# uurl/hivemq-mqtt-tensorflow-kafka-realtime-iot-machine-learning-training-inference

Hardware: AMD Instinct MI355X
Metric: sensor-rows/sec (autoencoder train) + p50 per-event inference µs at 1/2/4/8 MI355X (higher is better)
Workload: dtype bf16

## Files before the change

### hivemq-mqtt-tensorflow-kafka-realtime-iot-machine-learning-training-inference_amd/csrc/include/sml_ops.h

```cpp
#pragma once
#include <hip/hip_runtime.h>
#include <stdint.h>

namespace sml {

int ae_nslot();
int ae_train_blocks_per_cu();
int ae_nparam();
int ae_waves_per_block();
int ae_train_grid(int64_t n, int max_blocks);
hipError_t ae_train_launch(const float* x, int64_t n, int64_t ld, const float* scale, const float* shift,
                           const float* params, float* partials, int64_t* iter, const int64_t* cursor,
                           const int* dims, const int* acts, float l1, int want_acc, int grid, const uint8_t* xpack,
                           hipStream_t stream, int* grid_used,
                           unsigned xpack_live = 0);
hipError_t ae_forward_launch(const float* x, int64_t n, int64_t ld, const float* scale, const float* shift,
                             const float* params, float* recon, float* score, uint8_t* flag, float threshold,
                             const int* dims, const int* acts, int max_blocks, hipStream_t stream,
                             float* metrics = nullptr);
hipError_t reduce_adam_launch(const float* partials, int G, int S, int nparam, float* grad_out, float* params,
                              float* m, float* v, const int64_t* iter, float lr, float beta1, float beta2, float eps,
                              float gscale, float* metrics_acc, int flags, int64_t* cursor, int64_t cursor_step,
                              int64_t cursor_ring, hipStream_t stream);
int slab_adam_columns(int S);
// ... 90 lines not shown
                                 const float* h0, const float* c0, const float* W, const float* Uw, const float* b,
                                 float* dh0, float* dc0, float* partials, int64_t B, int T, int IN, int act,
                                 int dh_last_only, int64_t x_seq, int frag, hipStream_t st);
inline int lstm_fused_bwd_slabs(int64_t B, int U, int IN, bool dx, bool x_bf16, bool dh_last_only) {
  return lstm_split_applies(U, IN, dx, x_bf16, dh_last_only) ? lstm_split_grid(B) : lstm_fused_slabs(B, U, dx);
}
int lstm_head_partials(int64_t n, int N);
hipError_t lstm_head_launch(const void* h, int64_t ldh, const float* W, const float* b, const float* y, int64_t ldy,
                            void* dh, int64_t n, int N, float gscale, float* part, float* grad, const int* map,
                            float* acc, float* out, float div0, float div1, int64_t* counter, hipStream_t st);
bool lstm_fused_frag_supported(int U, int IN, bool x_bf16, bool want_dx);

hipError_t pack_tiles_argmax_launch(const float* x, int64_t n, int64_t ld, int D, const float* scale,
                                    const float* shift, uint8_t* out, hipStream_t stream,
                                    const int64_t* index = nullptr, uint64_t perm_key = 0, int64_t perm_n = 0,
                                    uint64_t live_mask = 0);
hipError_t perm_indices_launch(int64_t* out, int64_t start, int64_t count, int64_t n, uint64_t key,
                               hipStream_t stream);
hipError_t row_argmax_launch(const float* x, int64_t n, int64_t ld, int D, const float* scale, const float* shift,
                             uint8_t* out, hipStream_t stream);

hipError_t mlp_fwd_launch(const void* x, int x_u8, int64_t ldx, const float* W, const float* b, float* y, int M,
                          int K, int N, int relu, float keep, uint32_t seed, uint32_t step, hipStream_t st);
hipError_t mlp_bwd_data_launch(const float* dz, const float* W, const float* h, float* dh, int M, int N1, int N2,
                               float inv_keep, hipStream_t st);
hipError_t mlp_wgrad_launch(const void* x, int x_u8, int64_t ldx, const float* dy, float* out, int B, int K, int N,
                            hipStream_t st);
hipError_t mlp_dropout_mask_launch(float* out, int M, int N, float keep, uint32_t seed, uint32_t step,
                                   hipStream_t st);

int lstm_ref_train_params();
// ... 76 lines not shown
```

### hivemq-mqtt-tensorflow-kafka-realtime-iot-machine-learning-training-inference_amd/csrc/kernels/ae_fused.hip

```cpp
#include <cstdlib>

#include "sml_common.h"
#include "sml_adam.h"

using namespace sml;

namespace {

constexpr int WAVES = 4;
constexpr int OFF1 = 0, OFF2 = 512, OFF3 = 768, OFF4 = 1024;
constexpr int NPARAM = 1536;
constexpr int NSLOT = 1540;
constexpr int SLAB_BYTES = WAVES * NSLOT * 4;

struct AEArgs {
  const float* x;
  int64_t n;
  int64_t ld;
  const float* scale;
  const float* shift;
  const float* params;
  float* partials;
  int64_t* iter;
  const int64_t* cursor;
// ... 620 lines not shown
    dz4r1[u] = lds_transpose(dz4b1[u], scr + 9 * 512, c, g);
  }
  if constexpr (U == 1) {
    xr0[1] = xr1[1] = dz1r[1] = h1r[1] = dz2r[1] = h2r[1] = dz3r[1] = h3r[1] = dz4r0[1] = dz4r1[1] = zb;
  }
  acc1[0] = mfma32(xr0[0], xr0[1], dz1r[0], dz1r[1], acc1[0]);
  acc1[1] = mfma32(xr1[0], xr1[1], dz1r[0], dz1r[1], acc1[1]);
  acc2 = mfma32(h1r[0], h1r[1], dz2r[0], dz2r[1], acc2);
  acc3 = mfma32(h2r[0], h2r[1], dz3r[0], dz3r[1], acc3);
  acc4[0] = mfma32(h3r[0], h3r[1], dz4r0[0], dz4r0[1], acc4[0]);
  acc4[1] = mfma32(h3r[0], h3r[1], dz4r1[0], dz4r1[1], acc4[1]);
}

constexpr unsigned kLiveCardata = 0x3FFFFu & ~((1u << 0) | (1u << 2) | (1u << 4) | (1u << 5));
__host__ __device__ constexpr bool cm_dead(int f) { return f == 0 || f == 2 || f == 4 || f == 5; }
__device__ __forceinline__ int cm_off(int g) { return g < 2 ? 0 : g == 2 ? 16 : 32; }
__device__ __forceinline__ f32x4 cm_row_x(const char* row, int g) {
  typedef __attribute__((address_space(3))) const f32x2_t lds_f2;
  const f32x2_t a = *(lds_f2*)(row + cm_off(g)), b = *(lds_f2*)(row + cm_off(g) + 8);
  return f32x4{a[0], g == 0 ? a[0] : a[1], b[0], g == 0 ? a[1] : b[1]};
}
__device__ __forceinline__ f32x4 cm_zero_dead(f32x4 x, int g) {
  return f32x4{g < 2 ? 0.f : x[0], g == 1 ? 0.f : x[1], g == 0 ? 0.f : x[2], x[3]};
}

struct FragsP {
  bf16x4 w1t;
  bf16x4 w1u[2];
  bf16x4 w2t[2];
  bf16x4 w3t;
  bf16x4 w4t[2];
  bf16x4 w4u;
  bf16x4 w4b[2];
  bf16x4 w4bu;
  bf16x4 w3b;
  bf16x4 w2b[2];
  s16x8 w1a[2], w2a, w4ba, w4bua;
  s16x8 w1s;
};
// ... 121 lines not shown
    s1 = base + pin * w + 16 + 4 * (out - 16);
    s2 = base + (pin + 8) * w + 16 + 8 + 4 * (out - 16);
    return;
  }
  s1 = base + pin * w + out;
  s2 = base + (pin + 8) * w + out + (l3 ? 8 : 0);
}

__device__ __forceinline__ void tr_write(bf16x4 v, char* slot, int c, int g) {
  *(lds_bf16x4*)(slot + tr_wr_off(c, g)) = v;
}
__device__ __forceinline__ bf16x4 tr_read(char* slot, int c, int g) {
  return __builtin_amdgcn_ds_read_tr16_b64_v4i16((lds_bf16x4*)(slot + tr_rd_off(c, g)));
}

template <int PACK, int DC, bool TP, int TS = 10, int NP = 1, int XP = 0, bool RX = false, bool CM = false>
__device__ __forceinline__ void train_pair_packed(const AEArgs& a, const FragsP& F, char* scr, int c, int g,
                                                  const f32x4 (&xf)[NP][2][2], const float (&xup)[NP],
                                                  const int (&ix)[NP][2], f32x4 acc1[2], f32x4& acc2, f32x4& acc3,
                                                  f32x4 acc4[2], f32x4& acc2b, f32x4& acc4b, float& sq, float& ab,
                                                  float& corr, float& rows, const char* const* xring = nullptr) {
  static_assert(PACK == PACK_REF && DC == 18, "reference model, D = 18 (outputs 16, 17 packed as UP)");
  static_assert(NP == 1 || NP == 2, "one or two pairs per iteration");
  const f32x4 zero4 = {0.f, 0.f, 0.f, 0.f};
  const bf16x4 zb = {0, 0, 0, 0};
  const bool pad_lane = (g == 3);
  const bool lo = c < 8;
  auto stand_in = [](int p, int u) { return TP && p == NP - 1 && u == 1; };
  constexpr bool EW = XP == 1 || XP == 3, MA = XP >= 1, TRM = XP == 2;
  bf16x4 ident;
#pragma unroll
  for (int j = 0; j < 4; ++j) ident[j] = bfbits(4 * g + j == c ? 1.0f : 0.0f);
  auto mfma_tr = [&](bf16x4 v) -> bf16x4 { return pack4(mfma16(v, ident, zero4)); };

  bf16x4 xb0[NP][2], h1b[NP][2], xub[NP];
  f32x4 h1[NP][2], y[NP][2], z1[NP][2], l1s[NP][2];
#pragma unroll
  for (int p = 0; p < NP; ++p) {
#pragma unroll
    for (int u = 0; u < 2; ++u) xb0[p][u] = pack4(xf[p][u][0]);
    xub[p] = pack4(f32x4{xup[p], g == 0 ? 1.0f : 0.0f, 0.f, 0.f});
    if constexpr (EW) {
      tr_write(xb0[p][0], scr + (p * 10 + 0) * 512, c, g);
      tr_write(xb0[p][1], scr + (p * 10 + 1) * 512, c, g);
      tr_write(xub[p], scr + (p * 10 + 2) * 512, c, g);
    }
  }
#pragma unroll
  for (int p = 0; p < NP; ++p) {
    if constexpr (MA) {
      const bf16x4 xu0 = pack4(f32x4{g < 2 ? xup[p] : 0.f, g == 0 ? 1.0f : 0.0f, 0.f, 0.f});
      const bf16x4 xu1 = pack4(f32x4{g >= 2 ? xup[p] : 0.f, g == 0 ? 1.0f : 0.0f, 0.f, 0.f});
      z1[p][0] = mfma32a(F.w1s, xb0[p][0], xu0, zero4);
      z1[p][1] = mfma32a(F.w1s, xb0[p][1], xu1, zero4);
    } else {
      z1[p][0] = mfma32a(F.w1a[0], xb0[p][0], xub[p], zero4);
      z1[p][1] = mfma32a(F.w1a[1], xub[p], xb0[p][1], zero4);
    }
  }
#pragma unroll
  for (int p = 0; p < NP; ++p)
#pragma unroll
    for (int u = 0; u < 2; ++u) {
#pragma unroll
      for (int i = 0; i < 4; ++i) h1[p][u][i] = tanh_exp2(z1[p][u][i]);
      h1b[p][u] = pack4(h1[p][u]);
      if constexpr (EW) tr_write(h1b[p][u], scr + (p * 10 + 3 + u) * 512, c, g);
// ... 22 lines not shown
  for (int p = 0; p < NP; ++p) z3[p] = mfma16(F.w3t, h2b[p], zero4);
#pragma unroll
  for (int p = 0; p < NP; ++p) {
#pragma unroll
    for (int i = 0; i < 4; ++i) h3[p][i] = tanh_exp2(z3[p][i]);
    h3b[p] = pack4(h3[p]);
    if constexpr (EW) tr_write(h3b[p], scr + (p * 10 + 6) * 512, c, g);
  }
  f32x4 dz4[NP][2], z4[NP][2], z4u[NP];
  float dz4up[NP], yup[NP];
  f32x4 xl[NP][2];
  float xul[NP];
#pragma unroll
  for (int p = 0; p < NP; ++p) {
    if constexpr (RX) {
      typedef __attribute__((address_space(3))) const f32x2_t lds_f2;
      typedef __attribute__((address_space(3))) const float lds_f;
      constexpr int DR = CM ? 14 : 18, SLOTB = 64 * DR + 16;
#pragma unroll
      for (int u = 0; u < 2; ++u) {
        if constexpr (CM) {
          xl[p][u] = cm_row_x(xring[p] + u * SLOTB + c * 4 * DR, g);
        } else {
          const char* row = xring[p] + u * SLOTB + c * 4 * 18 + 16 * g;
          const f32x2_t v0 = *(lds_f2*)row, v1 = *(lds_f2*)(row + 8);
          xl[p][u] = f32x4{v0[0], v0[1], v1[0], v1[1]};
        }
      }
      xul[p] = *(lds_f*)(xring[p] + c * 4 * DR + 4 * (DR - 2 + (g & 1)) + (g >= 2 ? SLOTB : 0));
    } else {
#pragma unroll
      for (int u = 0; u < 2; ++u) xl[p][u] = xf[p][u][0];
      xul[p] = xup[p];
    }
    if constexpr (CM) {
#pragma unroll
      for (int u = 0; u < 2; ++u) xl[p][u] = cm_zero_dead(xl[p][u], g);
    }
  }
#pragma unroll
  for (int p = 0; p < NP; ++p) {
#pragma unroll
    for (int u = 0; u < 2; ++u) z4[p][u] = mfma16(F.w4t[u], h3b[p], zero4);
    z4u[p] = mfma16(F.w4u, h3b[p], zero4);
  }
#pragma unroll
  for (int p = 0; p < NP; ++p) {
#pragma unroll
    for (int u = 0; u < 2; ++u)
#pragma unroll
      for (int i = 0; i < 4; ++i) {
        y[p][u][i] = relu_fast(z4[p][u][i]);
        float e = y[p][u][i] - xl[p][u][i];
        if (stand_in(p, u)) e = 0.f;
        sq = fmaf(e, e, sq);
        dz4[p][u][i] = y[p][u][i] > 0.f ? e : 0.f;
      }
    yup[p] = relu_fast(z4u[p][0]);
    float eup = yup[p] - xul[p];
    if (TP && p == NP - 1) eup = g < 2 ? eup : 0.f;
    sq = fmaf(eup, eup, sq);
    dz4up[p] = yup[p] > 0.f ? eup : 0.f;
  }
  if (a.want_acc) {
#pragma unroll
    for (int p = 0; p < NP; ++p) {
      const int iy = row_argmax_up_pair(y[p][0], y[p][1], yup[p], g);
      const int sel = -(g & 1);
      const int ixs = (ix[p][0] & ~sel) | (ix[p][1] & sel);
      corr += (((TP && p == NP - 1) ? g == 0 : g < 2) && iy == ixs) ? 1.f : 0.f;
    }
  }
  rows += (g == 0) ? (TP ? 2.f * NP - 1.f : 2.f * NP) : 0.f;

  bf16x4 dz4b[NP][2], dz1b[NP][2], dz4bu[NP], dz3b[NP], dz2b[NP];
  f32x4 d3[NP], d2[NP];
#pragma unroll
  for (int p = 0; p < NP; ++p) {
#pragma unroll
    for (int u = 0; u < 2; ++u) dz4b[p][u] = pack4(dz4[p][u]);
    dz4bu[p] = pack4(f32x4{dz4up[p], 0.f, 0.f, 0.f});
  }
#pragma unroll
  for (int p = 0; p < NP; ++p) {
    d3[p] = mfma32a(F.w4ba, dz4b[p][0], dz4b[p][1], zero4);
    d3[p] = mfma32a(F.w4bua, dz4bu[p], zb, d3[p]);
  }
#pragma unroll
// ... 200 lines not shown
        if (lane < nl2) glds16(src + 1024, voff, dst + 1024);
      };
      constexpr int CH = XM == 3 ? 8 : 1;
      auto next_tile = [&](int64_t t) -> int64_t {
        if constexpr (CH == 1) return t + stride;
        return ((t + 1) & (CH - 1)) ? t + 1 : t + 1 + (stride - 1) * CH;
      };
      const int64_t t0 = ufirst * CH;
      if constexpr (ILP >= 2) {
        static_assert((XM == 1 || (XM == 0 && ILP == 3)) && CH == 1 && PF >= 3,
                      "tile pairs: tile-packed ring (or raw rows, packed pairs), plain order");
        auto ring_tile = [&](int slot, f32x4 xf[2], int& ix) {
          typedef __attribute__((address_space(3))) const unsigned char lds_u8;
          if constexpr (XM == 1) ix = (int)*(lds_u8*)(ring + slot * slotb + (slotb - 16) + c);
          if constexpr (CMP) {
            xf[0] = cm_row_x(ring + slot * slotb + c * 4 * DR, g);
            xf[1] = f32x4{0.f, 0.f, 0.f, 0.f};
            return;
          }
          if constexpr (ILP == 3) {
            typedef __attribute__((address_space(3))) const f32x2_t lds_f2;
            const char* row = ring + slot * slotb + c * 4 * a.D + 16 * g;
            const f32x2_t v0 = *(lds_f2*)row, v1 = *(lds_f2*)(row + 8);
            xf[0] = f32x4{v0[0], v0[1], v1[0], v1[1]};
            xf[1] = f32x4{0.f, 0.f, 0.f, 0.f};
            return;
          }
          ring_x(a, ring + slot * slotb, c, g, xf);
#pragma unroll
          for (int j = 0; j < 4; ++j) xf[1][j] = (live_hi<DC>(j) && 16 + 4 * g + j < DC) ? xf[1][j] : 0.f;
        };
        static_assert(ILP != 3 || PF % 2 == 0, "pairs start on even ring slots");
        const int up_off = c * 4 * DR + 4 * (DR - 2 + (g & 1)) + (g >= 2 ? slotb : 0);
        auto ring_up = [&](int slot) -> float {
          typedef __attribute__((address_space(3))) const float lds_f;
          return *(lds_f*)(ring + slot * slotb + up_off);
        };
        if constexpr (ILP == 3) {
          constexpr int PS = PF / 2, NVP = CMP ? 2 : 3;
          const int pairb = 2 * slotb;
          const int nl3 = (pairb - (CMP ? 1024 : 2048)) >> 4;
          const int64_t npairs = nfull >> 1;
          auto issue_pair = [&](int64_t pi, int ps) {
            pi = pi < npairs ? pi : npairs - 1;
            const char* src = (XM == 1 ? reinterpret_cast<const char*>(a.xpack) : reinterpret_cast<const char*>(a.x)) +
                              pi * pairb;
            const unsigned dst = ring_lds + ps * pairb;
            glds16(src, voff, dst);
            if constexpr (CMP) {
              if (lane < nl3) glds16(src + 1024, voff, dst + 1024);
            } else {
              glds16(src + 1024, voff, dst + 1024);
              if (lane < nl3) glds16(src + 2048, voff, dst + 2048);
            }
          };
          static_assert(PS > NPW, "ring: at least one pair in flight");
          auto load_pair = [&](int slot, f32x4 (&xf)[2][2], float& xup, int (&ix)[2]) {
            ring_tile(2 * slot, xf[0], ix[0]);
            ring_tile(2 * slot + 1, xf[1], ix[1]);
            xup = ring_up(2 * slot);
            if constexpr (XM == 0) {
              typedef __attribute__((address_space(3))) const f32x4 lds_f4;
              typedef __attribute__((address_space(3))) const float lds_f;
              const f32x4 nsc = *(lds_f4*)(norm + 16 * g), nsh = *(lds_f4*)(norm + 128 + 16 * g);
              const int fu = 4 * (16 + (g & 1));
              const float usc = *(lds_f*)(norm + fu), ush = *(lds_f*)(norm + 128 + fu);
#pragma unroll
              for (int u = 0; u < 2; ++u)
#pragma unroll
                for (int j = 0; j < 4; ++j) xf[u][0][j] = fmaf(xf[u][0][j], nsc[j], nsh[j]);
              xup = fmaf(xup, usc, ush);
              ix[0] = ix[1] = a.want_acc ? row_argmax_up_pair_signed(xf[0][0], xf[1][0], xup, g) : -1;
            }
          };
          int64_t pp = ufirst;
#pragma unroll
          for (int k = 0; k < PS - NPW; ++k) {
            issue_pair(pp, k);
            pp += stride;
          }
          int rs = 0, ws = PS - NPW;
          int64_t pi = ufirst;
          for (; pi + (NPW - 1) * stride < npairs; pi += NPW * stride) {
#pragma unroll
            for (int k = 0; k < NPW; ++k) {
              issue_pair(pp, ws);
              pp += stride;
              ws = ws + 1 == PS ? 0 : ws + 1;
            }
            asm volatile("s_waitcnt vmcnt(%0)" ::"n"(NVP * (PS - NPW)) : "memory");
            f32x4 xf[NPW][2][2];
            float xup[NPW];
            int ix[NPW][2];
            const char* xr[NPW];
#pragma unroll
            for (int k = 0; k < NPW; ++k) {
              load_pair(rs, xf[k], xup[k], ix[k]);
              xr[k] = ring + 2 * rs * slotb;
              rs = rs + 1 == PS ? 0 : rs + 1;
            }
            constexpr bool RX = XM == 1 && OCC >= 4;
            train_pair_packed<PACK, DC, false, TS, NPW, XP, RX, CMP>(a, FP, scr, c, g, xf, xup, ix, acc1, acc2, acc3,
                                                                     acc4, acc2b, acc4b, sq, ab, corr, rows, xr);
          }
          if (NPW == 2 && pi < npairs) {
            static_assert(NPW == 1 || PS - NPW - 1 >= 0, "ring depth");
            asm volatile("s_waitcnt vmcnt(%0)" ::"n"(NVP * (PS - NPW - 1)) : "memory");
            f32x4 xf[1][2][2];
            float xup[1];
            int ix[1][2];
            load_pair(rs, xf[0], xup[0], ix[0]);
            train_pair_packed<PACK, DC, false, TS, 1, XP, false, CMP>(a, FP, scr, c, g, xf, xup, ix, acc1, acc2, acc3,
                                                                      acc4, acc2b, acc4b, sq, ab, corr, rows);
          }
          asm volatile("s_waitcnt vmcnt(0)" ::: "memory");
        } else {
        int64_t tp = t0;
#pragma unroll
        for (int k = 0; k < PF - 2; ++k) {
          issue(tp, k);
          tp += stride;
        }
        int rd = 0, wr = PF - 2;
        int64_t t = t0;
        for (; t + stride < nfull; t += 2 * stride) {
          issue(tp, wr);
          issue(tp + stride, wr + 1 == PF ? 0 : wr + 1);
          tp += 2 * stride;
          asm volatile("s_waitcnt vmcnt(%0)" ::"n"(NV * (PF - 2)) : "memory");
          f32x4 xf[2][2];
// ... 498 lines not shown
  auto pair_grid = [&](int occ_pairs = 3) {
    static const int rounds = [] {
      const char* e = std::getenv("SML_AE_ROUNDS");
      const int r = e ? std::atoi(e) : 3;
      return r >= 1 && r <= 8 ? r : 3;
    }();
    set_grid(rounds * occ_pairs * device_cus());
  };
  if (pack == PACK_REF) {
    const bool xa_ok = xpack != nullptr && want_acc && (n & 15) == 0 &&
                       ((reinterpret_cast<uintptr_t>(xpack) & 15) == 0);
    static const int probe = [] {
      const char* e = std::getenv("SML_AE_XPROBE");
      return e ? std::atoi(e) : 0;
    }();
    const bool pairs_ok = ((n >> 4) & 1) == 0 && train_ilp() == 3 && dims[1] <= 15 && dims[2] <= 7 && dims[3] <= 7;
    const bool full = xpack_live == 0 || (D <= 31 && xpack_live == (1u << D) - 1u);
    const bool cm = !full && D == 18 && xpack_live == kLiveCardata;
    if (xpack != nullptr && !full && !cm) return hipErrorInvalidValue;
    const bool xpack_used = xa_ok && ring_ok && D == 18 && (cm ? pairs_ok : (train_ilp() == 2 || pairs_ok || occ == 4));
    if (xpack != nullptr && !xpack_used && (probe < 2 || cm)) return hipErrorInvalidValue;
    if (ring_ok && occ == 4 && D == 18 && want_acc && probe == 2)
      hipLaunchKernelGGL((ae_train_kernel<PACK_REF, true, 3, 4, 18, 2>), gd, bd, 0, stream, a);
    else if (ring_ok && occ == 4 && D == 18 && want_acc && probe == 3)
      hipLaunchKernelGGL((ae_train_kernel<PACK_REF, true, 3, 4, 18, 3>), gd, bd, 0, stream, a);
    else if (ring_ok && D == 18 && xa_ok && train_ilp() == 2) {
      pair_grid();
      hipLaunchKernelGGL((ae_train_kernel<PACK_REF, true, 6, 3, 18, 1, 2>), gd, bd, 0, stream, a);
    } else if (ring_ok && D == 18 && xa_ok && ((n >> 4) & 1) == 0 && train_ilp() == 3 && dims[1] <= 15 &&
               dims[2] <= 7 && dims[3] <= 7) {
// ... 118 lines not shown
```

### hivemq-mqtt-tensorflow-kafka-realtime-iot-machine-learning-training-inference_amd/csrc/kernels/preprocess.hip

```cpp
#include <algorithm>

#include "sml_common.h"

namespace {

constexpr int kThreads = 256;
constexpr int kWaves = kThreads / 64;
constexpr int kTilesPerWave = 8;
constexpr int kRowsPerGroup = 16 * kTilesPerWave;

__device__ __forceinline__ void wave_lds_sync() {
  asm volatile("s_waitcnt lgkmcnt(0)" ::: "memory");
  __builtin_amdgcn_wave_barrier();
}

__device__ __forceinline__ int64_t imin64(int64_t a, int64_t b) { return a < b ? a : b; }
__device__ __forceinline__ int64_t imax64(int64_t a, int64_t b) { return a > b ? a : b; }

__device__ __forceinline__ float4 ld4(const float* p) { return *reinterpret_cast<const float4*>(p); }

}

namespace sml {
__host__ __device__ __forceinline__ uint64_t perm_mix(uint64_t z) {
// ... 130 lines not shown

__device__ __forceinline__ void load_tables(float* s_sc, float* s_sh, int period, int D, const float* scale,
                                            const float* shift) {
  for (int p = threadIdx.x; p < period; p += kThreads) {
    const int col = p % D;
    s_sc[p] = scale ? scale[col] : 1.0f;
    s_sh[p] = scale ? shift[col] : 0.0f;
  }
}

template <int DT, bool CONTIG, int MODE>
__global__ __launch_bounds__(kThreads) void rows_group_kernel(const float* __restrict__ x, int64_t n, int64_t ld,
                                                              int Drt, const float* __restrict__ scale,
                                                              const float* __restrict__ shift,
                                                              uint8_t* __restrict__ out, RowSource src,
                                                              int vec2, uint64_t live) {
  const int D = DT > 0 ? DT : Drt;
  __shared__ int s_col[64];
  const int nlive = MODE == 2 ? __popcll(live) : D;
  if (MODE == 2 && threadIdx.x < 64) {
    int k = (int)threadIdx.x, col = 0;
    for (int f = 0; f < D; ++f)
      if ((live >> f) & 1) {
        if (k == 0) col = f;
        --k;
      }
    s_col[threadIdx.x] = col;
  }
  extern __shared__ __attribute__((aligned(16))) char smem[];
  const int period = 4 * D;
  float* s_sc = reinterpret_cast<float*>(smem);
  float* s_sh = s_sc + period;
  const int lane = threadIdx.x & 63, wid = threadIdx.x >> 6;
  const int srcw = src.gather() ? 2 * kRowsPerGroup : 0;
  float* stage = s_sh + period + wid * (kRowsPerGroup * D + 32 + srcw);
  uint8_t* s_arg = reinterpret_cast<uint8_t*>(stage + kRowsPerGroup * D);
  int64_t* s_src = reinterpret_cast<int64_t*>(stage + kRowsPerGroup * D + 32);
  load_tables(s_sc, s_sh, period, D, scale, shift);
  __syncthreads();
  const int tile_chunks = 4 * D;
  const int ctile_chunks = 4 * nlive;
// ... 49 lines not shown
  }
}

size_t rows_group_lds(int D, bool gather) {
  return (size_t)(8 * D + kWaves * (kRowsPerGroup * D + 32 + (gather ? 2 * kRowsPerGroup : 0))) * sizeof(float);
}

int stream_grid(int64_t groups_of_waves) {
  const int64_t cap = 256 * 8;
  return (int)std::max<int64_t>(1, std::min<int64_t>(cap, (groups_of_waves + kWaves - 1) / kWaves));
}

template <int MODE>
hipError_t launch_rows_group(const float* x, int64_t n, int64_t ld, int D, const float* scale, const float* shift,
                             uint8_t* out, hipStream_t stream, RowSource src = RowSource{nullptr, 0, 0, 0},
                             uint64_t live = 0) {
  const bool gather = src.index != nullptr || src.half > 0;
  const bool contig = !gather && ld == D && (reinterpret_cast<uintptr_t>(x) & 15) == 0;
  const int vec2 = (ld & 1) == 0 && (reinterpret_cast<uintptr_t>(x) & 7) == 0;
  const int64_t groups = (n + kRowsPerGroup - 1) / kRowsPerGroup;
  const dim3 grid(stream_grid(groups)), block(kThreads);
  const size_t lds = rows_group_lds(D, gather);
  if (lds > 160 * 1024) return hipErrorInvalidValue;
  if (lds > 65536) {
    hipError_t e = hipSuccess;
    if (D == 18 && contig)
      e = hipFuncSetAttribute(reinterpret_cast<const void*>(rows_group_kernel<18, true, MODE>),
                              hipFuncAttributeMaxDynamicSharedMemorySize, (int)lds);
    else if (contig)
      e = hipFuncSetAttribute(reinterpret_cast<const void*>(rows_group_kernel<0, true, MODE>),
                              hipFuncAttributeMaxDynamicSharedMemorySize, (int)lds);
    else if (D == 18)
      e = hipFuncSetAttribute(reinterpret_cast<const void*>(rows_group_kernel<18, false, MODE>),
                              hipFuncAttributeMaxDynamicSharedMemorySize, (int)lds);
    else
      e = hipFuncSetAttribute(reinterpret_cast<const void*>(rows_group_kernel<0, false, MODE>),
                              hipFuncAttributeMaxDynamicSharedMemorySize, (int)lds);
    if (e != hipSuccess) return e;
  }
  if (D == 18 && contig)
    hipLaunchKernelGGL((rows_group_kernel<18, true, MODE>), grid, block, lds, stream, x, n, ld, D, scale, shift, out,
                       src, vec2, live);
  else if (contig)
    hipLaunchKernelGGL((rows_group_kernel<0, true, MODE>), grid, block, lds, stream, x, n, ld, D, scale, shift, out,
                       src, vec2, live);
  else if (D == 18)
    hipLaunchKernelGGL((rows_group_kernel<18, false, MODE>), grid, block, lds, stream, x, n, ld, D, scale, shift, out,
                       src, vec2, live);
  else
    hipLaunchKernelGGL((rows_group_kernel<0, false, MODE>), grid, block, lds, stream, x, n, ld, D, scale, shift, out,
                       src, vec2, live);
  return hipGetLastError();
}

__global__ __launch_bounds__(256) void perm_indices_kernel(int64_t* __restrict__ out, int64_t start, int64_t count,
                                                           int64_t n, uint64_t key, int half) {
  const int64_t i = (int64_t)blockIdx.x * 256 + threadIdx.x;
  if (i < count) out[i] = sml::perm_row(start + i, n, key, half);
}

constexpr int kChunk = 4096;
constexpr int kScanThreads = 1024;

__device__ __forceinline__ bool keep_row(const uint8_t* labels, int64_t r, int keep) {
  return keep < 0 || labels[r] == (uint8_t)keep;
}
// ... 127 lines not shown
  const size_t lds = (size_t)(8 * D + 4 + kWaves * 64 + kWaves * 64 * D) * sizeof(float);
  if (D == 18 && contig)
    hipLaunchKernelGGL((filter_scatter_kernel<18, true>), dim3(blocks), dim3(kThreads), lds, stream, x, n, ld, D,
                       labels, keep, scale, shift, counts, out, out_index);
  else if (contig)
    hipLaunchKernelGGL((filter_scatter_kernel<0, true>), dim3(blocks), dim3(kThreads), lds, stream, x, n, ld, D,
                       labels, keep, scale, shift, counts, out, out_index);
  else
    hipLaunchKernelGGL((filter_scatter_kernel<0, false>), dim3(blocks), dim3(kThreads), lds, stream, x, n, ld, D,
                       labels, keep, scale, shift, counts, out, out_index);
  return hipGetLastError();
}

hipError_t pack_tiles_argmax_launch(const float* x, int64_t n, int64_t ld, int D, const float* scale,
                                    const float* shift, uint8_t* out, hipStream_t stream, const int64_t* index,
                                    uint64_t perm_key, int64_t perm_n, uint64_t live_mask) {
  if (n <= 0) return hipSuccess;
  if ((n & 15) || D < 1 || D > 64) return hipErrorInvalidValue;
  if (reinterpret_cast<uintptr_t>(out) & 15) return hipErrorInvalidValue;
  if (perm_n > 0 && (index != nullptr || n > perm_n)) return hipErrorInvalidValue;
  const RowSource src{index, perm_key, perm_n, perm_n > 0 ? perm_half_bits(perm_n) : 0};
  const uint64_t all = D == 64 ? ~0ull : (1ull << D) - 1ull;
  if (live_mask & ~all) return hipErrorInvalidValue;
  if (live_mask != 0 && live_mask != all)
    return launch_rows_group<2>(x, n, ld, D, scale, shift, out, stream, src, live_mask);
  return launch_rows_group<0>(x, n, ld, D, scale, shift, out, stream, src);
}

hipError_t perm_indices_launch(int64_t* out, int64_t start, int64_t count, int64_t n, uint64_t key,
                               hipStream_t stream) {
  if (count <= 0) return hipSuccess;
  if (n <= 0 || start < 0 || start + count > n) return hipErrorInvalidValue;
  hipLaunchKernelGGL(perm_indices_kernel, dim3((unsigned)((count + 255) / 256)), dim3(256), 0, stream, out, start,
                     count, n, key, perm_half_bits(n));
  return hipGetLastError();
}

hipError_t row_argmax_launch(const float* x, int64_t n, int64_t ld, int D, const float* scale, const float* shift,
                             uint8_t* out, hipStream_t stream) {
  if (n <= 0) return hipSuccess;
// ... 6 lines not shown
```

### hivemq-mqtt-tensorflow-kafka-realtime-iot-machine-learning-training-inference_amd/csrc/torch_bind.cpp

```cpp
#include <torch/extension.h>
#include <c10/hip/HIPStream.h>
#include <c10/hip/HIPGuard.h>
#include <hip/hip_runtime.h>

#include "sml_ops.h"
#include "../runtime/p2p.h"
#include "sml_p2p.h"
#include "sml_scorer_api.h"
#include "../runtime/ring.h"
#include "../runtime/serve.h"
#include "../runtime/stream_ring.h"
#include "../runtime/queues.h"

#include <pybind11/numpy.h>
#include <cstdlib>
#include <cstring>

namespace {

static bool sync_check() {
  const char* v = std::getenv("SML_SYNC_CHECK");
  return v && *v && *v != '0';
}

// ... 81 lines not shown
  TORCH_CHECK(partials.numel() >= (int64_t)grid * sml::ae_nslot(), "partials buffer too small for grid ", grid);
  int used = grid;
  c10::hip::HIPGuard guard(x.device().index());
  int d[4] = {(int)dims[0], (int)dims[1], (int)dims[2], (int)dims[3]};
  int a[4] = {(int)acts[0], (int)acts[1], (int)acts[2], (int)acts[3]};
  SML_CHECK_HIP(sml::ae_train_launch(x.data_ptr<float>(), n, x.stride(0), opt_ptr(scale), opt_ptr(shift),
                                     params.data_ptr<float>(), partials.data_ptr<float>(), iter_ptr, cur_ptr, d, a,
                                     (float)l1,
                                     want_acc ? 1 : 0, grid, xpack_ptr, cur_stream(x), &used, (unsigned)xpack_live));
  return used;
}

at::Tensor pack_tiles_argmax(const at::Tensor& x, int64_t D, const c10::optional<at::Tensor>& scale,
                             const c10::optional<at::Tensor>& shift, const c10::optional<at::Tensor>& index,
                             const c10::optional<at::Tensor>& out_opt, uint64_t perm_key, int64_t perm_n,
                             int64_t n_rows, uint64_t live_mask) {
  check_dev(x, "x", at::kFloat);
  TORCH_CHECK(x.dim() == 2 && x.stride(1) == 1 && x.size(1) >= D && D >= 1 && D <= 64,
              "x must be [n, >=D] with D <= 64");
  TORCH_CHECK(scale.has_value() == shift.has_value(), "scale and shift go together");
  if (scale.has_value()) TORCH_CHECK(scale->numel() >= D && shift->numel() >= D, "scale/shift too short");
  int64_t n = x.size(0);
  const int64_t* idx = nullptr;
  if (index.has_value() && index->defined()) {
    TORCH_CHECK(index->is_cuda() && index->device() == x.device() && index->scalar_type() == at::kLong &&
                    index->dim() == 1 && index->is_contiguous(), "index must be a contiguous int64 device vector");
    n = index->numel();
    if (n > 0) {
      const auto mm = at::aminmax(*index);
      TORCH_CHECK(std::get<0>(mm).item<int64_t>() >= 0 && std::get<1>(mm).item<int64_t>() < x.size(0),
                  "index out of range for x");
    }
    idx = index->data_ptr<int64_t>();
  }
  if (perm_n > 0) {
    TORCH_CHECK(idx == nullptr, "index and perm are exclusive");
    TORCH_CHECK(perm_n <= x.size(0), "perm_n larger than x");
    n = n_rows >= 0 ? n_rows : perm_n;
    TORCH_CHECK(n <= perm_n, "more packed rows than the permuted domain");
  } else if (n_rows >= 0) {
    TORCH_CHECK(n_rows <= n, "n_rows larger than the source");
    n = n_rows;
  }
  TORCH_CHECK(n % 16 == 0, "packed rows must be a multiple of 16");
  const uint64_t all = D == 64 ? ~0ull : (1ull << D) - 1ull;
  TORCH_CHECK((live_mask & ~all) == 0, "live_mask has bits past D");
  const int64_t cols = live_mask ? __builtin_popcountll(live_mask) : D;
  const int64_t bytes = n / 16 * (64 * cols + 16);
  c10::hip::HIPGuard guard(x.device().index());
  at::Tensor out;
  if (out_opt.has_value() && out_opt->defined()) {
    out = *out_opt;
    TORCH_CHECK(out.is_cuda() && out.device() == x.device() && out.scalar_type() == at::kByte && out.is_contiguous() &&
                    out.numel() >= bytes && (reinterpret_cast<uintptr_t>(out.data_ptr()) & 15) == 0,
                "out must be a contiguous, 16-byte aligned uint8 device buffer of >= the packed size");
  } else {
    out = at::empty({bytes}, x.options().dtype(at::kByte));
  }
  SML_CHECK_HIP(sml::pack_tiles_argmax_launch(x.data_ptr<float>(), n, x.stride(0), (int)D, opt_ptr(scale),
                                              opt_ptr(shift), out.data_ptr<uint8_t>(), cur_stream(x), idx, perm_key,
                                              perm_n, live_mask));
  return out;
}

at::Tensor perm_indices(const at::Tensor& like, int64_t n, uint64_t key, int64_t start, int64_t count) {
  TORCH_CHECK(like.is_cuda(), "like must be a device tensor");
  if (count < 0) count = n - start;
  TORCH_CHECK(n > 0 && start >= 0 && count >= 0 && start + count <= n, "need 0 <= start, start + count <= n");
  c10::hip::HIPGuard guard(like.device().index());
  auto out = at::empty({count}, like.options().dtype(at::kLong));
  SML_CHECK_HIP(sml::perm_indices_launch(out.data_ptr<int64_t>(), start, count, n, key, cur_stream(like)));
  return out;
}

at::Tensor row_argmax_u8(const at::Tensor& x, int64_t D, const c10::optional<at::Tensor>& scale,
                         const c10::optional<at::Tensor>& shift) {
// ... 1162 lines not shown

}

PYBIND11_MODULE(TORCH_EXTENSION_NAME, m) {
  m.doc() = "streamml gfx950 HIP kernels";
  m.attr("AE_NSLOT") = sml::ae_nslot();
  m.attr("AE_NPARAM") = sml::ae_nparam();
  m.def("ae_train_partials", &ae_train_partials, "fused AE fwd+bwd -> per-workgroup gradient slabs",
        py::arg("x"), py::arg("scale"), py::arg("shift"), py::arg("params"), py::arg("partials"), py::arg("iter"),
        py::arg("dims"), py::arg("acts"), py::arg("l1"), py::arg("want_acc"), py::arg("max_blocks"),
        py::arg("n_rows") = -1, py::arg("cursor") = py::none(), py::arg("xpack") = py::none(),
        py::arg("xpack_live") = 0);
  m.def("pack_tiles_argmax", &pack_tiles_argmax, "tile-packed training ring (rows + ingest-time argmax per tile)",
        py::arg("x"), py::arg("D"), py::arg("scale") = py::none(), py::arg("shift") = py::none(),
        py::arg("index") = py::none(), py::arg("out") = py::none(), py::arg("perm_key") = 0,
        py::arg("perm_n") = 0, py::arg("n_rows") = -1, py::arg("live_mask") = 0);
  m.def("perm_indices", &perm_indices, "the pack's keyed row bijection of [0, n), materialised", py::arg("like"),
        py::arg("n"), py::arg("key"), py::arg("start") = 0, py::arg("count") = -1);
  m.def("row_argmax_u8", &row_argmax_u8, "ingest-time argmax of each normalised row (uint8)", py::arg("x"),
        py::arg("D"), py::arg("scale") = py::none(), py::arg("shift") = py::none());
  m.def("ae_minibatch_max_batch", &sml::ae_minibatch_max_batch, "largest batch the persistent small-batch trainer takes");
  m.def("ae_train_minibatches", &ae_train_minibatches,
        "persistent small-batch AE trainer: nsteps sequential Keras steps (fwd+bwd+Adam) in one launch",
        py::arg("x"), py::arg("cursor"), py::arg("scale"), py::arg("shift"), py::arg("params"), py::arg("m"),
        py::arg("v"), py::arg("iter"), py::arg("metrics"), py::arg("batch"), py::arg("nsteps"), py::arg("dims"),
        py::arg("acts"), py::arg("l1"), py::arg("lr"), py::arg("beta1"), py::arg("beta2"), py::arg("eps"),
        py::arg("gscale"), py::arg("want_acc"), py::arg("prof") = py::none(), py::arg("lrs") = py::none(),
        py::arg("dp_peers") = 0, py::arg("dp_ranks") = 1, py::arg("dp_rank0") = 0, py::arg("dp_status") = 0,
        py::arg("dp_timeout_ticks") = 0, py::arg("ragged") = py::none(), py::arg("precision") = -1);
  m.def("normalize_filter", &normalize_filter, "K8: normalise + keep rows with label == keep, order-preserving",
        py::arg("x"), py::arg("D"), py::arg("labels"), py::arg("keep"), py::arg("scale"), py::arg("shift"),
// ... 173 lines not shown
```

### hivemq-mqtt-tensorflow-kafka-realtime-iot-machine-learning-training-inference_amd/ops/ae.py

```python
from __future__ import annotations


import os

from dataclasses import dataclass
from typing import List, Optional, Sequence, Tuple

import numpy as np
import torch

from ._ext import load_c

ACT_CODES = {"linear": 0, None: 0, "relu": 1, "tanh": 2, "sigmoid": 3}
NPARAM = 1536
NSLOT = 1540
LAYOUT = [(0, 32, 16, 31), (512, 16, 16, 15), (768, 16, 16, 15), (1024, 16, 32, 15)]

RA_WRITE_GRAD, RA_ADAM, RA_METRICS, RA_ADVANCE = 1, 2, 4, 8


def default_train_blocks(device) -> int:
    try:
        cus = torch.cuda.get_device_properties(torch.device(device)).multi_processor_count
    except Exception:
# ... 136 lines not shown
                           self.cursor, int(self.ring_batch), int(ring),
                           self.reduce_scratch if partials is None else None,
                           self.reduce_counters if partials is None else None)

    def attach_ring(self, ring: torch.Tensor, batch: int) -> None:
        self._check_x(ring)
        if batch <= 0 or ring.size(0) % batch:
            raise ValueError("ring rows must be a positive multiple of the batch")
        self.ring, self.ring_batch = ring, int(batch)
        self.cursor.zero_()
        self.ring_xpack = None
        self.ring_live = 0
        if self._xpack_ok(ring.size(0), batch) and ring.size(1) == self.spec.input_dim:
            self.ring_live = self._compact_mask(batch)
            self.ring_xpack = self.C.pack_tiles_argmax(ring, self.spec.input_dim, self.scale, self.shift,
                                                       live_mask=self.ring_live)

    COMPACT_LIVE = 0x3FFFF & ~((1 << 0) | (1 << 2) | (1 << 4) | (1 << 5))

    def _compact_mask(self, batch: int) -> int:
        if os.environ.get("SML_AE_COMPACT", "1") == "0" or os.environ.get("SML_AE_ILP", "3")[:1] in ("1", "2"):
            return 0
        if (batch // 16) % 2 or self.spec.encoding_dim > 15 or self.spec.hidden_dim > 7:
            return 0
        return self._norm_live if self._norm_live == self.COMPACT_LIVE else 0

    def _xpack_ok(self, rows: int, batch: int) -> bool:
        return (self.want_acc and os.environ.get("SML_AE_XPACK", "1") != "0" and rows % 16 == 0
                and batch % 16 == 0 and self.spec.input_dim == 18
                and tuple(self.spec.activations) == ("tanh", "relu", "tanh", "relu"))

# ... 7 lines not shown
            raise ValueError(f"fewer rows ({n}) than one batch ({B})")
        if not (self._xpack_ok(rows, B) and x.size(1) == self.spec.input_dim):
            if perm_key is not None:
                index = self.perm_indices(int(x.size(0)), perm_key)
            src = x[index[:rows]] if index is not None else x[:rows]
            self.attach_ring(src.contiguous(), B)
            return rows
        live = self._compact_mask(B)
        nbytes = rows // 16 * (64 * (bin(live).count("1") if live else self.spec.input_dim) + 16)
        buf = getattr(self, "_pack_buf", None)
        if not reuse or buf is None or buf.numel() < nbytes:
            buf = self._pack_buf = torch.empty(nbytes, dtype=torch.uint8, device=self.device)
        if perm_key is not None:
            self.C.pack_tiles_argmax(x, self.spec.input_dim, self.scale, self.shift, None, buf,
                                     perm_key=int(perm_key) & ((1 << 64) - 1), perm_n=int(x.size(0)), n_rows=rows,
                                     live_mask=live)
        else:
            idx = index[:rows].contiguous() if index is not None else None
            self.C.pack_tiles_argmax(x if idx is not None else x[:rows], self.spec.input_dim, self.scale, self.shift,
                                     idx, buf, live_mask=live)
        self.ring, self.ring_batch = x[:rows], B
        self.ring_xpack = buf[:nbytes]
        self.ring_live = live
        self.cursor.zero_()
        return rows

    def perm_indices(self, n: int, perm_key: int, start: int = 0, count: Optional[int] = None) -> torch.Tensor:
        return self.C.perm_indices(self.params, int(n), int(perm_key) & ((1 << 64) - 1), int(start),
                                   -1 if count is None else int(count))

    def step_ring(self, global_batch: Optional[int] = None, allreduce=None) -> None:
        if self.ring is None:
            raise RuntimeError("attach_ring() first")
        B = self.ring_batch
        gb = B if global_batch is None else int(global_batch)
# ... 192 lines not shown
```

Measured before the change: 53.31 billion.

## Store compact ring in lane order and add specialised two-slot ring loop

```diff
diff --git a/hivemq-mqtt-tensorflow-kafka-realtime-iot-machine-learning-training-inference_amd/csrc/include/sml_ops.h b/hivemq-mqtt-tensorflow-kafka-realtime-iot-machine-learning-training-inference_amd/csrc/include/sml_ops.h
--- a/hivemq-mqtt-tensorflow-kafka-realtime-iot-machine-learning-training-inference_amd/csrc/include/sml_ops.h
+++ b/hivemq-mqtt-tensorflow-kafka-realtime-iot-machine-learning-training-inference_amd/csrc/include/sml_ops.h
@@ -128,7 +128,7 @@
 hipError_t pack_tiles_argmax_launch(const float* x, int64_t n, int64_t ld, int D, const float* scale,
                                     const float* shift, uint8_t* out, hipStream_t stream,
                                     const int64_t* index = nullptr, uint64_t perm_key = 0, int64_t perm_n = 0,
-                                    uint64_t live_mask = 0);
+                                    uint64_t live_mask = 0, bool lane_order = false);
 hipError_t perm_indices_launch(int64_t* out, int64_t start, int64_t count, int64_t n, uint64_t key,
                                hipStream_t stream);
 hipError_t row_argmax_launch(const float* x, int64_t n, int64_t ld, int D, const float* scale, const float* shift,
diff --git a/hivemq-mqtt-tensorflow-kafka-realtime-iot-machine-learning-training-inference_amd/csrc/kernels/ae_fused.hip b/hivemq-mqtt-tensorflow-kafka-realtime-iot-machine-learning-training-inference_amd/csrc/kernels/ae_fused.hip
--- a/hivemq-mqtt-tensorflow-kafka-realtime-iot-machine-learning-training-inference_amd/csrc/kernels/ae_fused.hip
+++ b/hivemq-mqtt-tensorflow-kafka-realtime-iot-machine-learning-training-inference_amd/csrc/kernels/ae_fused.hip
@@ -658,15 +658,19 @@
 
 constexpr unsigned kLiveCardata = 0x3FFFFu & ~((1u << 0) | (1u << 2) | (1u << 4) | (1u << 5));
 __host__ __device__ constexpr bool cm_dead(int f) { return f == 0 || f == 2 || f == 4 || f == 5; }
-__device__ __forceinline__ int cm_off(int g) { return g < 2 ? 0 : g == 2 ? 16 : 32; }
-__device__ __forceinline__ f32x4 cm_row_x(const char* row, int g) {
+__device__ __forceinline__ int cm_off(int g) { return max(16 * g - 8, 0); }
+typedef __attribute__((address_space(3))) const char lds_cc;
+__device__ __forceinline__ f32x4 ring_row4(lds_cc* lane_row) {
   typedef __attribute__((address_space(3))) const f32x2_t lds_f2;
-  const f32x2_t a = *(lds_f2*)(row + cm_off(g)), b = *(lds_f2*)(row + cm_off(g) + 8);
-  return f32x4{a[0], g == 0 ? a[0] : a[1], b[0], g == 0 ? a[1] : b[1]};
-}
-__device__ __forceinline__ f32x4 cm_zero_dead(f32x4 x, int g) {
-  return f32x4{g < 2 ? 0.f : x[0], g == 1 ? 0.f : x[1], g == 0 ? 0.f : x[2], x[3]};
-}
+  const f32x2_t a = *(lds_f2*)lane_row, b = *(lds_f2*)(lane_row + 8);
+  return f32x4{a[0], a[1], b[0], b[1]};
+}
+__device__ __forceinline__ f32x4 cm_row_x(const char* lane_row) { return ring_row4((lds_cc*)lane_row); }
+
+template <int V>
+struct RingSlot {
+  static constexpr int value = V;
+};
 
 struct FragsP {
   bf16x4 w1t;
@@ -818,12 +822,14 @@
   return __builtin_amdgcn_ds_read_tr16_b64_v4i16((lds_bf16x4*)(slot + tr_rd_off(c, g)));
 }
 
-template <int PACK, int DC, bool TP, int TS = 10, int NP = 1, int XP = 0, bool RX = false, bool CM = false>
+template <int PACK, int DC, bool TP, int TS = 10, int NP = 1, int XP = 0, bool RX = false, bool CM = false,
+          bool WA = false, bool RC = true>
 __device__ __forceinline__ void train_pair_packed(const AEArgs& a, const FragsP& F, char* scr, int c, int g,
                                                   const f32x4 (&xf)[NP][2][2], const float (&xup)[NP],
                                                   const int (&ix)[NP][2], f32x4 acc1[2], f32x4& acc2, f32x4& acc3,
                                                   f32x4 acc4[2], f32x4& acc2b, f32x4& acc4b, float& sq, float& ab,
-                                                  float& corr, float& rows, const char* const* xring = nullptr) {
+                                                  float& corr, float& rows, lds_cc* const* xrow = nullptr,
+                                                  lds_cc* const* xupa = nullptr) {
   static_assert(PACK == PACK_REF && DC == 18, "reference model, D = 18 (outputs 16, 17 packed as UP)");
   static_assert(NP == 1 || NP == 2, "one or two pairs per iteration");
   const f32x4 zero4 = {0.f, 0.f, 0.f, 0.f};
@@ -853,8 +859,11 @@
 #pragma unroll
   for (int p = 0; p < NP; ++p) {
     if constexpr (MA) {
-      const bf16x4 xu0 = pack4(f32x4{g < 2 ? xup[p] : 0.f, g == 0 ? 1.0f : 0.0f, 0.f, 0.f});
-      const bf16x4 xu1 = pack4(f32x4{g >= 2 ? xup[p] : 0.f, g == 0 ? 1.0f : 0.0f, 0.f, 0.f});
+      typedef unsigned u32x2 __attribute__((ext_vector_type(2)));
+      const unsigned xw = __builtin_bit_cast(u32x2, xub[p])[0];
+      const unsigned bias_w = __float_as_uint(g == 0 ? 1.0f : 0.0f);
+      const bf16x4 xu0 = __builtin_bit_cast(bf16x4, u32x2{g < 2 ? xw : 0u, 0u});
+      const bf16x4 xu1 = __builtin_bit_cast(bf16x4, u32x2{g >= 2 ? xw : bias_w, 0u});
       z1[p][0] = mfma32a(F.w1s, xb0[p][0], xu0, zero4);
       z1[p][1] = mfma32a(F.w1s, xb0[p][1], xu1, zero4);
     } else {
@@ -907,30 +916,18 @@
 #pragma unroll
   for (int p = 0; p < NP; ++p) {
     if constexpr (RX) {
-      typedef __attribute__((address_space(3))) const f32x2_t lds_f2;
       typedef __attribute__((address_space(3))) const float lds_f;
       constexpr int DR = CM ? 14 : 18, SLOTB = 64 * DR + 16;
 #pragma unroll
-      for (int u = 0; u < 2; ++u) {
-        if constexpr (CM) {
-          xl[p][u] = cm_row_x(xring[p] + u * SLOTB + c * 4 * DR, g);
-        } else {
-          const char* row = xring[p] + u * SLOTB + c * 4 * 18 + 16 * g;
-          const f32x2_t v0 = *(lds_f2*)row, v1 = *(lds_f2*)(row + 8);
-          xl[p][u] = f32x4{v0[0], v0[1], v1[0], v1[1]};
-        }
-      }
-      xul[p] = *(lds_f*)(xring[p] + c * 4 * DR + 4 * (DR - 2 + (g & 1)) + (g >= 2 ? SLOTB : 0));
+      for (int u = 0; u < 2; ++u) xl[p][u] = ring_row4(xrow[p] + u * SLOTB);
+      xul[p] = *(lds_f*)xupa[p];
     } else {
 #pragma unroll
       for (int u = 0; u < 2; ++u) xl[p][u] = xf[p][u][0];
       xul[p] = xup[p];
     }
-    if constexpr (CM) {
-#pragma unroll
-      for (int u = 0; u < 2; ++u) xl[p][u] = cm_zero_dead(xl[p][u], g);
-    }
-  }
+  }
+  const float cm_m[3] = {g < 2 ? 0.f : 1.f, g == 1 ? 0.f : 1.f, g == 0 ? 0.f : 1.f};
 #pragma unroll
   for (int p = 0; p < NP; ++p) {
 #pragma unroll
@@ -944,7 +941,7 @@
 #pragma unroll
       for (int i = 0; i < 4; ++i) {
         y[p][u][i] = relu_fast(z4[p][u][i]);
-        float e = y[p][u][i] - xl[p][u][i];
+        float e = (CM && i < 3) ? fmaf(-xl[p][u][i], cm_m[i], y[p][u][i]) : y[p][u][i] - xl[p][u][i];
         if (stand_in(p, u)) e = 0.f;
         sq = fmaf(e, e, sq);
         dz4[p][u][i] = y[p][u][i] > 0.f ? e : 0.f;
@@ -955,7 +952,7 @@
     sq = fmaf(eup, eup, sq);
     dz4up[p] = yup[p] > 0.f ? eup : 0.f;
   }
-  if (a.want_acc) {
+  if (WA || a.want_acc) {
 #pragma unroll
     for (int p = 0; p < NP; ++p) {
       const int iy = row_argmax_up_pair(y[p][0], y[p][1], yup[p], g);
@@ -964,7 +961,7 @@
       corr += (((TP && p == NP - 1) ? g == 0 : g < 2) && iy == ixs) ? 1.f : 0.f;
     }
   }
-  rows += (g == 0) ? (TP ? 2.f * NP - 1.f : 2.f * NP) : 0.f;
+  if constexpr (RC) rows += (g == 0) ? (TP ? 2.f * NP - 1.f : 2.f * NP) : 0.f;
 
   bf16x4 dz4b[NP][2], dz1b[NP][2], dz4bu[NP], dz3b[NP], dz2b[NP];
   f32x4 d3[NP], d2[NP];
@@ -1195,7 +1192,7 @@
           typedef __attribute__((address_space(3))) const unsigned char lds_u8;
           if constexpr (XM == 1) ix = (int)*(lds_u8*)(ring + slot * slotb + (slotb - 16) + c);
           if constexpr (CMP) {
-            xf[0] = cm_row_x(ring + slot * slotb + c * 4 * DR, g);
+            xf[0] = cm_row_x(ring + slot * slotb + c * 4 * DR + cm_off(g));
             xf[1] = f32x4{0.f, 0.f, 0.f, 0.f};
             return;
           }
@@ -1212,7 +1209,8 @@
           for (int j = 0; j < 4; ++j) xf[1][j] = (live_hi<DC>(j) && 16 + 4 * g + j < DC) ? xf[1][j] : 0.f;
         };
         static_assert(ILP != 3 || PF % 2 == 0, "pairs start on even ring slots");
-        const int up_off = c * 4 * DR + 4 * (DR - 2 + (g & 1)) + (g >= 2 ? slotb : 0);
+        const int row_off = c * 4 * DR + (CMP ? cm_off(g) : 16 * g);
+        const int up_off = c * 4 * DR + (CMP ? 8 * (g & 1) : 4 * (DR - 2 + (g & 1))) + (g >= 2 ? slotb : 0);
         auto ring_up = [&](int slot) -> float {
           typedef __attribute__((address_space(3))) const float lds_f;
           return *(lds_f*)(ring + slot * slotb + up_off);
@@ -1222,8 +1220,7 @@
           const int pairb = 2 * slotb;
           const int nl3 = (pairb - (CMP ? 1024 : 2048)) >> 4;
           const int64_t npairs = nfull >> 1;
-          auto issue_pair = [&](int64_t pi, int ps) {
-            pi = pi < npairs ? pi : npairs - 1;
+          auto issue_pair_at = [&](int64_t pi, int ps) {
             const char* src = (XM == 1 ? reinterpret_cast<const char*>(a.xpack) : reinterpret_cast<const char*>(a.x)) +
                               pi * pairb;
             const unsigned dst = ring_lds + ps * pairb;
@@ -1235,6 +1232,10 @@
               if (lane < nl3) glds16(src + 2048, voff, dst + 2048);
             }
           };
+          auto issue_pair = [&](int64_t pi, int ps) {
+            issue_pair_at(pi < npairs ? pi : npairs - 1, ps);
+          };
+          (void)issue_pair;
           static_assert(PS > NPW, "ring: at least one pair in flight");
           auto load_pair = [&](int slot, f32x4 (&xf)[2][2], float& xup, int (&ix)[2]) {
             ring_tile(2 * slot, xf[0], ix[0]);
@@ -1254,6 +1255,52 @@
               ix[0] = ix[1] = a.want_acc ? row_argmax_up_pair_signed(xf[0][0], xf[1][0], xup, g) : -1;
             }
           };
+          (void)load_pair;
+          if constexpr (NPW == 1 && XM == 1 && PS == 2) {
+            const unsigned np32 = (unsigned)npairs, st32 = (unsigned)stride, uf32 = (unsigned)ufirst;
+            const unsigned ntrip = __builtin_amdgcn_readfirstlane(uf32 < np32 ? (np32 - 1u - uf32) / st32 + 1u : 0u);
+            unsigned pq = uf32;
+            auto issue_next = [&](int ps) {
+              issue_pair_at(pq < np32 ? pq : np32 - 1u, ps);
+              pq += st32;
+            };
+#pragma unroll
+            for (int k = 0; k < PS - 1; ++k) issue_next(k);
+            lds_cc* rowb = (lds_cc*)(ring + row_off);
+            lds_cc* upb = (lds_cc*)(ring + up_off);
+            lds_cc* axb = (lds_cc*)(ring + (slotb - 16) + c);
+            asm volatile("" : "+v"(rowb), "+v"(upb));
+            asm volatile("" : "+v"(axb));
+            auto trip = [&](auto slot) {
+              constexpr int rs = decltype(slot)::value, ws = (rs + PS - 1) % PS;
+              issue_next(ws);
+              asm volatile("s_waitcnt vmcnt(%0)" ::"n"(NVP * (PS - 1)) : "memory");
+              typedef __attribute__((address_space(3))) const unsigned char lds_u8;
+              typedef __attribute__((address_space(3))) const float lds_f;
+              f32x4 xf[1][2][2];
+              float xup[1];
+              int ix[1][2];
+              lds_cc* const xr[1] = {rowb + 2 * rs * slotb};
+              lds_cc* const xu[1] = {upb + 2 * rs * slotb};
+#pragma unroll
+              for (int u = 0; u < 2; ++u) {
+                xf[0][u][0] = ring_row4(xr[0] + u * slotb);
+                xf[0][u][1] = f32x4{0.f, 0.f, 0.f, 0.f};
+                ix[0][u] = (int)*(lds_u8*)(axb + (2 * rs + u) * slotb);
+              }
+              xup[0] = *(lds_f*)xu[0];
+              constexpr bool RX = OCC >= 4;
+              train_pair_packed<PACK, DC, false, TS, 1, XP, RX, CMP, true, false>(
+                  a, FP, scr, c, g, xf, xup, ix, acc1, acc2, acc3, acc4, acc2b, acc4b, sq, ab, corr, rows, xr, xu);
+            };
+            for (unsigned k = ntrip; k > 0; k -= PS) {
+              trip(RingSlot<0>{});
+              if (k == 1) break;
+              trip(RingSlot<1>{});
+            }
+            rows += (g == 0) ? 2.f * (float)ntrip : 0.f;
+            asm volatile("s_waitcnt vmcnt(0)" ::: "memory");
+          } else {
           int64_t pp = ufirst;
 #pragma unroll
           for (int k = 0; k < PS - NPW; ++k) {
@@ -1273,16 +1320,19 @@
             f32x4 xf[NPW][2][2];
             float xup[NPW];
             int ix[NPW][2];
-            const char* xr[NPW];
+            lds_cc* xr[NPW];
+            lds_cc* xu[NPW];
 #pragma unroll
             for (int k = 0; k < NPW; ++k) {
               load_pair(rs, xf[k], xup[k], ix[k]);
-              xr[k] = ring + 2 * rs * slotb;
+              xr[k] = (lds_cc*)(ring + 2 * rs * slotb + row_off);
+              xu[k] = (lds_cc*)(ring + 2 * rs * slotb + up_off);
               rs = rs + 1 == PS ? 0 : rs + 1;
             }
             constexpr bool RX = XM == 1 && OCC >= 4;
-            train_pair_packed<PACK, DC, false, TS, NPW, XP, RX, CMP>(a, FP, scr, c, g, xf, xup, ix, acc1, acc2, acc3,
-                                                                     acc4, acc2b, acc4b, sq, ab, corr, rows, xr);
+            train_pair_packed<PACK, DC, false, TS, NPW, XP, RX, CMP, XM == 1>(a, FP, scr, c, g, xf, xup, ix, acc1, acc2,
+                                                                              acc3, acc4, acc2b, acc4b, sq, ab, corr,
+                                                                              rows, xr, xu);
           }
           if (NPW == 2 && pi < npairs) {
             static_assert(NPW == 1 || PS - NPW - 1 >= 0, "ring depth");
@@ -1291,10 +1341,12 @@
             float xup[1];
             int ix[1][2];
             load_pair(rs, xf[0], xup[0], ix[0]);
-            train_pair_packed<PACK, DC, false, TS, 1, XP, false, CMP>(a, FP, scr, c, g, xf, xup, ix, acc1, acc2, acc3,
-                                                                      acc4, acc2b, acc4b, sq, ab, corr, rows);
+            train_pair_packed<PACK, DC, false, TS, 1, XP, false, CMP, XM == 1>(a, FP, scr, c, g, xf, xup, ix, acc1, acc2,
+                                                                               acc3, acc4, acc2b, acc4b, sq, ab, corr,
+                                                                               rows);
           }
           asm volatile("s_waitcnt vmcnt(0)" ::: "memory");
+          }
         } else {
         int64_t tp = t0;
 #pragma unroll
@@ -1823,6 +1875,7 @@
       const char* e = std::getenv("SML_AE_XPROBE");
       return e ? std::atoi(e) : 0;
     }();
+    if ((n >> 5) >= (int64_t(1) << 30)) return hipErrorInvalidValue;
     const bool pairs_ok = ((n >> 4) & 1) == 0 && train_ilp() == 3 && dims[1] <= 15 && dims[2] <= 7 && dims[3] <= 7;
     const bool full = xpack_live == 0 || (D <= 31 && xpack_live == (1u << D) - 1u);
     const bool cm = !full && D == 18 && xpack_live == kLiveCardata;
diff --git a/hivemq-mqtt-tensorflow-kafka-realtime-iot-machine-learning-training-inference_amd/csrc/kernels/preprocess.hip b/hivemq-mqtt-tensorflow-kafka-realtime-iot-machine-learning-training-inference_amd/csrc/kernels/preprocess.hip
--- a/hivemq-mqtt-tensorflow-kafka-realtime-iot-machine-learning-training-inference_amd/csrc/kernels/preprocess.hip
+++ b/hivemq-mqtt-tensorflow-kafka-realtime-iot-machine-learning-training-inference_amd/csrc/kernels/preprocess.hip
@@ -168,7 +168,7 @@
                                                               int Drt, const float* __restrict__ scale,
                                                               const float* __restrict__ shift,
                                                               uint8_t* __restrict__ out, RowSource src,
-                                                              int vec2, uint64_t live) {
+                                                              int vec2, uint64_t live, int lane_order) {
   const int D = DT > 0 ? DT : Drt;
   __shared__ int s_col[64];
   const int nlive = MODE == 2 ? __popcll(live) : D;
@@ -179,6 +179,10 @@
         if (k == 0) col = f;
         --k;
       }
+    if (lane_order) {
+      k = (int)threadIdx.x;
+      col = k == 0 ? 16 : k == 2 ? 17 : k < 4 ? k : k < 14 ? k + 2 : 0;
+    }
     s_col[threadIdx.x] = col;
   }
   extern __shared__ __attribute__((aligned(16))) char smem[];
@@ -258,7 +262,7 @@
 template <int MODE>
 hipError_t launch_rows_group(const float* x, int64_t n, int64_t ld, int D, const float* scale, const float* shift,
                              uint8_t* out, hipStream_t stream, RowSource src = RowSource{nullptr, 0, 0, 0},
-                             uint64_t live = 0) {
+                             uint64_t live = 0, int lane_order = 0) {
   const bool gather = src.index != nullptr || src.half > 0;
   const bool contig = !gather && ld == D && (reinterpret_cast<uintptr_t>(x) & 15) == 0;
   const int vec2 = (ld & 1) == 0 && (reinterpret_cast<uintptr_t>(x) & 7) == 0;
@@ -284,16 +288,16 @@
   }
   if (D == 18 && contig)
     hipLaunchKernelGGL((rows_group_kernel<18, true, MODE>), grid, block, lds, stream, x, n, ld, D, scale, shift, out,
-                       src, vec2, live);
+                       src, vec2, live, lane_order);
   else if (contig)
     hipLaunchKernelGGL((rows_group_kernel<0, true, MODE>), grid, block, lds, stream, x, n, ld, D, scale, shift, out,
-                       src, vec2, live);
+                       src, vec2, live, lane_order);
   else if (D == 18)
     hipLaunchKernelGGL((rows_group_kernel<18, false, MODE>), grid, block, lds, stream, x, n, ld, D, scale, shift, out,
-                       src, vec2, live);
+                       src, vec2, live, lane_order);
   else
     hipLaunchKernelGGL((rows_group_kernel<0, false, MODE>), grid, block, lds, stream, x, n, ld, D, scale, shift, out,
-                       src, vec2, live);
+                       src, vec2, live, lane_order);
   return hipGetLastError();
 }
 
@@ -451,7 +455,7 @@
 
 hipError_t pack_tiles_argmax_launch(const float* x, int64_t n, int64_t ld, int D, const float* scale,
                                     const float* shift, uint8_t* out, hipStream_t stream, const int64_t* index,
-                                    uint64_t perm_key, int64_t perm_n, uint64_t live_mask) {
+                                    uint64_t perm_key, int64_t perm_n, uint64_t live_mask, bool lane_order) {
   if (n <= 0) return hipSuccess;
   if ((n & 15) || D < 1 || D > 64) return hipErrorInvalidValue;
   if (reinterpret_cast<uintptr_t>(out) & 15) return hipErrorInvalidValue;
@@ -459,8 +463,10 @@
   const RowSource src{index, perm_key, perm_n, perm_n > 0 ? perm_half_bits(perm_n) : 0};
   const uint64_t all = D == 64 ? ~0ull : (1ull << D) - 1ull;
   if (live_mask & ~all) return hipErrorInvalidValue;
+  constexpr uint64_t kLaneOrderLive = 0x3FFFFull & ~((1ull << 0) | (1ull << 2) | (1ull << 4) | (1ull << 5));
+  if (lane_order && (D != 18 || live_mask != kLaneOrderLive)) return hipErrorInvalidValue;
   if (live_mask != 0 && live_mask != all)
-    return launch_rows_group<2>(x, n, ld, D, scale, shift, out, stream, src, live_mask);
+    return launch_rows_group<2>(x, n, ld, D, scale, shift, out, stream, src, live_mask, lane_order ? 1 : 0);
   return launch_rows_group<0>(x, n, ld, D, scale, shift, out, stream, src);
 }
 
diff --git a/hivemq-mqtt-tensorflow-kafka-realtime-iot-machine-learning-training-inference_amd/csrc/torch_bind.cpp b/hivemq-mqtt-tensorflow-kafka-realtime-iot-machine-learning-training-inference_amd/csrc/torch_bind.cpp
--- a/hivemq-mqtt-tensorflow-kafka-realtime-iot-machine-learning-training-inference_amd/csrc/torch_bind.cpp
+++ b/hivemq-mqtt-tensorflow-kafka-realtime-iot-machine-learning-training-inference_amd/csrc/torch_bind.cpp
@@ -119,7 +119,7 @@
 at::Tensor pack_tiles_argmax(const at::Tensor& x, int64_t D, const c10::optional<at::Tensor>& scale,
                              const c10::optional<at::Tensor>& shift, const c10::optional<at::Tensor>& index,
                              const c10::optional<at::Tensor>& out_opt, uint64_t perm_key, int64_t perm_n,
-                             int64_t n_rows, uint64_t live_mask) {
+                             int64_t n_rows, uint64_t live_mask, bool lane_order) {
   check_dev(x, "x", at::kFloat);
   TORCH_CHECK(x.dim() == 2 && x.stride(1) == 1 && x.size(1) >= D && D >= 1 && D <= 64,
               "x must be [n, >=D] with D <= 64");
@@ -150,6 +150,7 @@
   TORCH_CHECK(n % 16 == 0, "packed rows must be a multiple of 16");
   const uint64_t all = D == 64 ? ~0ull : (1ull << D) - 1ull;
   TORCH_CHECK((live_mask & ~all) == 0, "live_mask has bits past D");
+  TORCH_CHECK(!lane_order || (D == 18 && live_mask == 0x3FFCAull), "lane_order: D = 18 and the cardata live set only");
   const int64_t cols = live_mask ? __builtin_popcountll(live_mask) : D;
   const int64_t bytes = n / 16 * (64 * cols + 16);
   c10::hip::HIPGuard guard(x.device().index());
@@ -164,7 +165,7 @@
   }
   SML_CHECK_HIP(sml::pack_tiles_argmax_launch(x.data_ptr<float>(), n, x.stride(0), (int)D, opt_ptr(scale),
                                               opt_ptr(shift), out.data_ptr<uint8_t>(), cur_stream(x), idx, perm_key,
-                                              perm_n, live_mask));
+                                              perm_n, live_mask, lane_order));
   return out;
 }
 
@@ -1357,7 +1358,8 @@
   m.def("pack_tiles_argmax", &pack_tiles_argmax, "tile-packed training ring (rows + ingest-time argmax per tile)",
         py::arg("x"), py::arg("D"), py::arg("scale") = py::none(), py::arg("shift") = py::none(),
         py::arg("index") = py::none(), py::arg("out") = py::none(), py::arg("perm_key") = 0,
-        py::arg("perm_n") = 0, py::arg("n_rows") = -1, py::arg("live_mask") = 0);
+        py::arg("perm_n") = 0, py::arg("n_rows") = -1, py::arg("live_mask") = 0,
+        py::arg("lane_order") = false);
   m.def("perm_indices", &perm_indices, "the pack's keyed row bijection of [0, n), materialised", py::arg("like"),
         py::arg("n"), py::arg("key"), py::arg("start") = 0, py::arg("count") = -1);
   m.def("row_argmax_u8", &row_argmax_u8, "ingest-time argmax of each normalised row (uint8)", py::arg("x"),
diff --git a/hivemq-mqtt-tensorflow-kafka-realtime-iot-machine-learning-training-inference_amd/ops/ae.py b/hivemq-mqtt-tensorflow-kafka-realtime-iot-machine-learning-training-inference_amd/ops/ae.py
--- a/hivemq-mqtt-tensorflow-kafka-realtime-iot-machine-learning-training-inference_amd/ops/ae.py
+++ b/hivemq-mqtt-tensorflow-kafka-realtime-iot-machine-learning-training-inference_amd/ops/ae.py
@@ -174,7 +174,7 @@
         if self._xpack_ok(ring.size(0), batch) and ring.size(1) == self.spec.input_dim:
             self.ring_live = self._compact_mask(batch)
             self.ring_xpack = self.C.pack_tiles_argmax(ring, self.spec.input_dim, self.scale, self.shift,
-                                                       live_mask=self.ring_live)
+                                                       live_mask=self.ring_live, lane_order=self.ring_live != 0)
 
     COMPACT_LIVE = 0x3FFFF & ~((1 << 0) | (1 << 2) | (1 << 4) | (1 << 5))
 
@@ -212,11 +212,11 @@
         if perm_key is not None:
             self.C.pack_tiles_argmax(x, self.spec.input_dim, self.scale, self.shift, None, buf,
                                      perm_key=int(perm_key) & ((1 << 64) - 1), perm_n=int(x.size(0)), n_rows=rows,
-                                     live_mask=live)
+                                     live_mask=live, lane_order=live != 0)
         else:
             idx = index[:rows].contiguous() if index is not None else None
             self.C.pack_tiles_argmax(x if idx is not None else x[:rows], self.spec.input_dim, self.scale, self.shift,
-                                     idx, buf, live_mask=live)
+                                     idx, buf, live_mask=live, lane_order=live != 0)
         self.ring, self.ring_batch = x[:rows], B
         self.ring_xpack = buf[:nbytes]
         self.ring_live = live
```

After: 55.55 billion, median of 6. 4.2% higher.
